# nebarnix/Project-Desert-Tortoise

Hardware: AMD Instinct MI355X
Metric: IQ Msamples/s end-to-end (WAV→minorframes), 1-GPU + %HBM roofline (higher is better)
Workload: dtype f32

## Files before the change

include/pdt_dev.h:

```cpp
#ifndef PDT_DEV_H
#define PDT_DEV_H
#include <stdint.h>
#ifdef __cplusplus
extern "C" {
#endif
int pdt_dev_set(const char *name, const char *value);
struct pdt_ctx;
unsigned long long pdt_dev_span_rows(const struct pdt_ctx *ctx, unsigned *n_exits_out, unsigned long long max);
int pdt_dev_ddc(int device, uint32_t in_rate, int decim, double offset_hz, int sample_format, const void *x_dev, long long lo, long long hi,
                uint64_t n_out, uint64_t g0, void *out_dev);
#ifdef __cplusplus
}
#endif
#endif
```

project-desert-tortoise_amd/__init__.py:

```python
from __future__ import annotations

import collections
import ctypes as C
import os
import struct

import numpy as np

_HERE = os.path.dirname(os.path.abspath(__file__))
LIBPDT_PATH = os.environ.get("PDT_LIBPDT_PATH") or os.path.join(_HERE, "csrc", "libpdt.so")
LIBSYNTH_PATH = os.path.join(_HERE, "synth", "libpdtsynth.so")

MODE_POES, MODE_ARGOS = 0, 1
SAMPLER_GARDNER, SAMPLER_MM = 0, 1
CHAIN_FILE, CHAIN_LIVE = 0, 1
ST_PLL, ST_LOCK, ST_FIR, ST_AGC, ST_SYM, ST_SYMIDX, ST_BITS, ST_BITSYM, ST_AGC_RAW, ST_ANALYTIC, ST_CHANNEL = range(11)
FMT_PCM16, FMT_F32, FMT_REAL_PCM16, FMT_REAL_F32 = range(4)


FMT_WB_PCM16, FMT_WB_F32, FMT_WB_CU8, FMT_WB_CS8 = range(16, 20)


class PdtError(RuntimeError):
    pass
# ... 238 lines not shown
    "pdt_demod_pcm16", "pdt_demod_device", "pdt_demod_f32", "pdt_demod_device_f32", "pdt_demod_batch_device", "pdt_num_frames", "pdt_frames", "pdt_get_stats",
    "pdt_format_frames", "pdt_read_stage", "pdt_stage_len", "pdt_kernel_times", "pdt_make_lpf",
    "pdt_wav_parse_header", "pdt_time_axis", "pdt_stage_bytesync", "pdt_tip_check", "pdt_tip_frames",
    "pdt_stream_begin", "pdt_stream_push_pcm16", "pdt_stream_push_f32", "pdt_stream_end", "pdt_stream_frames",
    "pdt_keep_quality", "pdt_chunk_reports", "pdt_stage_manchester", "pdt_stage_fir", "pdt_stage_agc", "pdt_stage_squelch", "pdt_stage_pll", "pdt_stage_gardner", "pdt_stage_static_gain", "pdt_stage_mm",
    "pdt_keep_presquelch", "pdt_keep_pll", "pdt_stage_bytesync_from", "pdt_demod_fd", "pdt_format_records", "pdt_stream_retained", "pdt_host_math", "pdt_get_device",
    "pdt_write_frames", "pdt_write_records", "pdt_demod_file", "pdt_set_loop_params", "pdt_set_progress",
    "pdt_set_real_input", "pdt_demod_real", "pdt_demod_device_real", "pdt_stream_push_real", "pdt_host_analytic",
    "pdt_set_channel", "pdt_demod_channel", "pdt_demod_device_channel", "pdt_demod_channels_device", "pdt_demod_channels", "pdt_stream_push_channel", "pdt_host_ddc",
    "pdt_survey", "pdt_survey_device", "pdt_survey_spectrum", "pdt_host_survey",
    "pdt_bursts", "pdt_bursts_device", "pdt_burst_carriers", "pdt_waterfall_rows", "pdt_bursts_shape", "pdt_burst_peaks", "pdt_host_bursts",
    "pdt_device_math", "pdt_device_math_layout",
    "pdt_burst_windows", "pdt_demod_windows_device", "pdt_demod_windows", "pdt_demod_windows_held",
    "pdt_tones", "pdt_tones_batch", "pdt_host_tones",
]
DEV_SYMBOLS = ["pdt_dev_set", "pdt_dev_span_rows", "pdt_dev_ddc"]

_lib = None


def _share_torch_hip_runtime():
    import importlib.util
    import sys
    if "torch" in sys.modules:
        return
    try:
        spec = importlib.util.find_spec("torch")
    except (ImportError, ValueError):
        return
    if spec is None or not spec.submodule_search_locations:
        return
# ... 77 lines not shown
    L.pdt_stage_fir.argtypes = [C.c_void_p, C.c_void_p, C.c_uint64, C.c_void_p, C.c_void_p]
    L.pdt_stage_fir.restype = C.c_int
    L.pdt_keep_quality.argtypes = [C.c_void_p, C.c_int]
    L.pdt_keep_quality.restype = C.c_int
    L.pdt_keep_pll.argtypes = [C.c_void_p, C.c_int]
    L.pdt_keep_pll.restype = C.c_int
    L.pdt_chunk_reports.argtypes = [C.c_void_p, C.c_void_p, C.c_uint64]
    L.pdt_chunk_reports.restype = C.c_uint64
    L.pdt_set_progress.argtypes = [C.c_void_p, C.c_void_p, C.c_void_p]
    L.pdt_tip_check.argtypes = [C.c_void_p, C.POINTER(TipSummary)]
    L.pdt_tip_frames.argtypes = [C.c_void_p, C.c_void_p, C.c_uint64]
    L.pdt_tip_frames.restype = C.c_uint64
    L.pdt_write_frames.argtypes = [C.c_void_p, C.c_int, C.POINTER(C.c_uint64)]
    L.pdt_write_records.argtypes = [C.c_void_p, C.c_uint64, C.c_int, C.POINTER(C.c_uint64)]
    L.pdt_dev_set.argtypes = [C.c_char_p, C.c_char_p]
    L.pdt_set_loop_params.argtypes = [C.c_void_p, C.POINTER(LoopParams)]
    L.pdt_demod_file.argtypes = [C.c_void_p, C.c_int, C.c_uint64, C.c_uint64, C.c_int, C.c_int, C.POINTER(C.c_uint64)]
    L.pdt_set_real_input.argtypes = [C.c_void_p, C.c_double]
    L.pdt_demod_real.argtypes = [C.c_void_p, C.c_void_p, C.c_uint64, C.c_int]
    L.pdt_demod_device_real.argtypes = [C.c_void_p, C.c_void_p, C.c_uint64, C.c_int]
    L.pdt_stream_push_real.argtypes = [C.c_void_p, C.c_void_p, C.c_uint64, C.c_int, C.POINTER(C.c_uint64)]
    L.pdt_host_analytic.argtypes = [C.c_uint32, C.c_double, C.c_void_p, C.c_uint64, C.c_int, C.c_void_p]
    L.pdt_set_channel.argtypes = [C.c_void_p, C.c_int, C.c_double]
    L.pdt_demod_channel.argtypes = [C.c_void_p, C.c_void_p, C.c_uint64, C.c_int]
    L.pdt_demod_device_channel.argtypes = [C.c_void_p, C.c_void_p, C.c_uint64, C.c_int]
    L.pdt_demod_channels_device.argtypes = [C.POINTER(C.c_void_p), C.c_int, C.c_void_p, C.c_uint64, C.c_int]
    L.pdt_demod_channels.argtypes = [C.POINTER(C.c_void_p), C.c_int, C.c_void_p, C.c_uint64, C.c_int]
    L.pdt_stream_push_channel.argtypes = [C.c_void_p, C.c_void_p, C.c_uint64, C.c_int, C.POINTER(C.c_uint64)]
    L.pdt_host_ddc.argtypes = [C.c_uint32, C.c_int, C.c_double, C.c_void_p, C.c_uint64, C.c_int, C.c_void_p]
    L.pdt_dev_ddc.argtypes = [C.c_int, C.c_uint32, C.c_int, C.c_double, C.c_int, C.c_void_p, C.c_longlong, C.c_longlong, C.c_uint64, C.c_uint64, C.c_void_p]
# ... 326 lines not shown
        c, cap = _tone_cfg(cfg)
        out, count = np.zeros(max(cap, 1), dtype=TONE_DTYPE), C.c_int(0)
        _check(self._L.pdt_tones(self._h, C.byref(c) if c else None, out.ctypes.data, cap, C.byref(count)), "pdt_tones")
        return out[:count.value]

    def device_math(self, fn: int, records: np.ndarray) -> np.ndarray:
        dt, nin, nout = device_math_layout(fn)
        a = np.ascontiguousarray(records)
        if a.dtype != dt or a.size % nin:
            raise PdtError(f"pdt_device_math({fn}): records of {nin} x {dt} wanted, got {a.dtype} x {a.shape}")
        n = a.size // nin
        out = np.empty((n, nout), dtype=dt)
        _check(self._L.pdt_device_math(self._h, fn, a.ctypes.data, n, out.ctypes.data), "pdt_device_math")
        return out

    def demod_device(self, dev_ptr: int, nframes: int):
        _check(self._L.pdt_demod_device(self._h, C.c_void_p(dev_ptr), nframes), "pdt_demod_device")
        return self

    def bytesync(self, bits: np.ndarray):
        b = np.ascontiguousarray(bits, dtype=np.uint8)
        _check(self._L.pdt_stage_bytesync(self._h, b.ctypes.data, b.size), "pdt_stage_bytesync")
        return self

    def _dt(self):
        return np.dtype("<f8") if (self.mode == MODE_ARGOS and not self.chain) else np.dtype("<f4")

    def stage_manchester(self, symbols: np.ndarray, resync_threshold: float, state: "ManchesterState | None" = None):
        a = np.ascontiguousarray(symbols, dtype=self._dt())
        bits = np.zeros(a.size + 4, dtype=np.uint8)
# ... 315 lines not shown
```

project-desert-tortoise_amd/csrc/pdt_api.hip:

```cpp
#include "pdt_rt.h"
#include "pdt_analytic.h"
#include "pdt_ddc.h"
#include "pdt_survey.h"
#include "pdt_bursts.h"
#include "pdt_tone.h"

#include <pthread.h>
#include <sched.h>
#include <sys/mman.h>
#include <sys/stat.h>
#include <sys/syscall.h>

namespace pdtrt {
PDT_CHAIN_INSTANCES(extern, float)
PDT_CHAIN_INSTANCES(extern, double)
std::atomic<long long> g_alloc_ns{0};
hipError_t analytic_launch(hipStream_t st, int fmt, const void *x, long long lo, long long hi, unsigned long long n_out, unsigned long long g0,
                           uint32_t step, const float *tab_dev, void *out);
size_t survey_part_floats(uint64_t nseg, int nfft);
hipError_t survey_launch(hipStream_t st, int fmt, const void *x, uint64_t nseg, int nfft, const float *win, const float *tw, float *part, float *out);
int survey_plan(const pdt_survey_cfg *cfg, double mode_range_hz, double channel_rate, uint64_t nframes, int cap, pdt::SurveyPlan *p);
int survey_carriers(const float *P, const pdt::SurveyPlan &p, double in_rate, pdt_carrier *found);
hipError_t waterfall_launch(hipStream_t st, int fmt, const void *x, uint64_t nrows, int rows_per, int nfft, const float *win, const float *tw, float *rows);
hipError_t row_peaks_launch(hipStream_t st, const float *rows, uint64_t nrows, int nfft, float level, int gb, void *peaks, int *counts);
// ... 30 lines not shown
    if (const char *e = get("PDT_PLL_BLOCK")) pll_block = atoi(e);
    if (const char *e = get("PDT_HBM_LIMIT_MB")) hbm_limit_mb = std::max(1ll, atoll(e));
    if (const char *e = get("PDT_BURST_SLAB_ROWS")) burst_slab_rows = std::max(1ll, atoll(e));
    if (const char *e = get("PDT_WINDOW_PIECE")) window_piece = std::max(1ll, atoll(e));
    if (const char *e = get("PDT_SCOUT_SYMS")) scout_syms = std::max(16, atoi(e));
    if (const char *e = get("PDT_FIR_WG_PER_CU")) fir_wg_per_cu = std::min(4096, std::max(1, atoi(e)));
    if (const char *e = get("PDT_INGEST_THREADS")) ingest_threads = std::min(128, std::max(1, atoi(e)));
    if (const char *e = get("PDT_INGEST_SPAN_MB")) ingest_span_mb = std::min(256, std::max(1, atoi(e)));
    if (const char *e = get("PDT_INGEST_STREAMS")) ingest_streams = std::min(4, std::max(1, atoi(e)));
    if (const char *e = get("PDT_INGEST_DIRECT")) ingest_direct = atoi(e) ? 1 : 0;
    if (const char *e = get("PDT_INGEST_NUMA")) ingest_numa = atoi(e) ? 1 : 0;
    if (const char *e = get("PDT_FIX_PASSES")) fix_passes = atoi(e);
    if (const char *e = get("PDT_GSEG")) gseg = std::min(64, std::max(2, atoi(e)));
    if (const char *e = get("PDT_GSPAN")) gspan = std::min(256, std::max(1, atoi(e)));
    if (const char *e = get("PDT_GSPAN_CAP")) gspan_cap = std::max(64, atoi(e));
    fir_generic = get("PDT_FIR_GENERIC") != nullptr;
    mix_unfused = get("PDT_MIX_UNFUSED") != nullptr;
    quality_inline = get("PDT_QUALITY_INLINE") != nullptr;
    gardner_nostride = get("PDT_GARDNER_NOSTRIDE") != nullptr;
    gemit_groups = get("PDT_GEMIT_GROUPS") != nullptr;
    agc_unfused = get("PDT_AGC_UNFUSED") != nullptr;
    manch_3pass = get("PDT_MANCH_3PASS") != nullptr;
    sync_serial = get("PDT_SYNC_SERIAL") != nullptr;
    agc_lanes = get("PDT_AGC_LANES") != nullptr;
    no_excl = get("PDT_NO_EXCL") != nullptr;
    gardner_onebuf = get("PDT_GARDNER_ONEBUF") != nullptr;
    gardner_noring = get("PDT_GARDNER_NORING") != nullptr;
    ema_noguess = get("PDT_EMA_NOGUESS") != nullptr;
    gardner_sequential = get("PDT_GARDNER_SEQUENTIAL") != nullptr;
    seg_sequential = get("PDT_SEG_SEQUENTIAL") != nullptr;
// ... 575 lines not shown
{
    if (!ctx || ctx->gspan_nrows <= 0 || !ctx->gspan_rows.p) return 0;
    const unsigned long long n = (unsigned long long)ctx->gspan_nrows, m = std::min(n, max);
    if (n_exits_out && m) {
        std::vector<GardnerSpanRow> rows((size_t)m);
        if (hipSetDevice(ctx->cfg.device) != hipSuccess ||
            hipMemcpy(rows.data(), ctx->gspan_rows.p, (size_t)m * sizeof(GardnerSpanRow), hipMemcpyDeviceToHost) != hipSuccess) {
            (void)hipGetLastError();
            return 0;
        }
        for (size_t k = 0; k < (size_t)m; k++) n_exits_out[k] = rows[k].n;
    }
    return n;
}

int pdt_dev_ddc(int device, uint32_t in_rate, int decim, double offset_hz, int sample_format, const void *x_dev, long long lo, long long hi,
                uint64_t n_out, uint64_t g0, void *out_dev)
{
    if (in_rate == 0 || decim < DDC_MIN_DECIM || decim > DDC_MAX_DECIM || !ddc_fmt(sample_format) || !x_dev || !out_dev) return PDT_ERR_ARG;
    if (!(std::isfinite(offset_hz) && std::fabs(offset_hz) < 0.5 * (double)in_rate)) return PDT_ERR_ARG;
    HIP_TRY(hipSetDevice(device));
    const std::vector<float> taps = ddc_taps(decim);
    std::vector<float> tab(2 * AN_TAB);
    analytic_table(tab.data());
    DevBuf dtaps, dtab;
    auto run = [&]() -> int {
        int rc;
        if ((rc = dtaps.ensure(taps.size() * sizeof(float) + 16)) || (rc = dtab.ensure(tab.size() * sizeof(float) + 16))) return rc;
        HIP_TRY(hipMemcpy(dtaps.p, taps.data(), taps.size() * sizeof(float), hipMemcpyHostToDevice));
        HIP_TRY(hipMemcpy(dtab.p, tab.data(), tab.size() * sizeof(float), hipMemcpyHostToDevice));
// ... 192 lines not shown
    if (argos_twin) ctx->axis_f.init(1 / (float)cfg->sample_rate);
    ctx->axis_d.init(1.0 / (double)cfg->sample_rate);
    ctx->counted = true;
    g_open_contexts.fetch_add(1);
    *out = ctx;
    return PDT_OK;
}

void pdt_close(pdt_ctx *ctx)
{
    if (!ctx) return;
    (void)hipSetDevice(ctx->cfg.device);
    DevBuf *bufs[] = { &ctx->pcm, &ctx->pll, &ctx->lock, &ctx->fir, &ctx->agc, &ctx->sym, &ctx->symidx, &ctx->bits, &ctx->bitsym,
                       &ctx->hits, &ctx->frames, &ctx->taps, &ctx->mag, &ctx->seams_pll, &ctx->seams_agc, &ctx->scal, &ctx->lockinfo,
                       &ctx->term, &ctx->seams_ema, &ctx->gtable, &ctx->gentries, &ctx->gcand,
                       &ctx->gmfirst, &ctx->stiles, &ctx->gsegmap, &ctx->gsegstart, &ctx->gbands, &ctx->gclist, &ctx->gspan_keys, &ctx->gspan_tails, &ctx->gspan_rows, &ctx->gspan_items, &ctx->gspan_ctl, &ctx->gspan_recs, &ctx->gcentries, &ctx->gflags, &ctx->agc_maps, &ctx->pll_head, &ctx->taps_rot, &ctx->pll_scratch, &ctx->tip, &ctx->stream_in, &ctx->sync_scr, &ctx->agc_raw, &ctx->agc_ckpt, &ctx->pll_ckpt, &ctx->packs_dev, &ctx->seg_dev, &ctx->lt_theta, &ctx->lt_phi,
                       &ctx->avgph, &ctx->term_ap, &ctx->seams_q, &ctx->chunkinfo, &ctx->an_tab, &ctx->analytic, &ctx->halo.buf[0], &ctx->halo.buf[1],
                       &ctx->ddc_taps, &ctx->channel, &ctx->survey_win, &ctx->survey_tw, &ctx->survey_part, &ctx->survey_out,
                       &ctx->bursts_rows, &ctx->bursts_peaks, &ctx->bursts_counts, &ctx->win_table, &ctx->tone_table, &ctx->tone_out };
    for (DevBuf *b : bufs) b->release();
    for (hipEvent_t e : ctx->event_pool) (void)hipEventDestroy(e);
    if (ctx->pinned) (void)hipHostFree(ctx->pinned);
    if (ctx->qual_pin) (void)hipHostFree(ctx->qual_pin);
    if (ctx->packs_pin) (void)hipHostFree(ctx->packs_pin);
    if (ctx->ingest_pin) (void)hipHostFree(ctx->ingest_pin);
    for (hipEvent_t e : ctx->ingest_ev) (void)hipEventDestroy(e);
    if (ctx->ev_ingest) (void)hipEventDestroy(ctx->ev_ingest);
    if (ctx->copy_stream) (void)hipStreamDestroy(ctx->copy_stream);
    for (hipEvent_t e : ctx->span_ev) (void)hipEventDestroy(e);
    for (int q = 0; q < 3; q++) {
        if (ctx->ev_ingest_more[q]) (void)hipEventDestroy(ctx->ev_ingest_more[q]);
// ... 1743 lines not shown
```

project-desert-tortoise_amd/csrc/pdt_chain.inc:

```
#include "pdt_rt.h"

namespace pdtrt {
PDT_WIDE_INSTANCES(extern, float)
PDT_WIDE_INSTANCES(extern, double)

template <typename T> int finish_capture(pdt_ctx *ctx, uint64_t n, const FinishArgs &FA)
{
    const bool argos = FA.argos, need_lock = FA.need_lock, fuse_mix = FA.fuse_mix;
    const long long N = FA.N, n_out = FA.n_out, chunk = FA.chunk, chunk_out = FA.chunk_out, first = FA.first, first_out = FA.first_out,
                    sym_cap = FA.sym_cap;
    const int interp = FA.interp, ntaps = FA.ntaps;
    const uint32_t hit_cap = FA.hit_cap, frame_cap = FA.frame_cap;
    const SyncParams &SP = FA.SP;
    const T Fs = (T)ctx->cfg.sample_rate;
    StreamCarry *seg = ctx->sc.active ? &ctx->sc : nullptr;
    FrameRec *d_frames = (FrameRec *)ctx->frames.p;
    (void)first_out;
    if (!ctx->pending || ctx->pend_n != n) return PDT_ERR_STATE;
    ctx->pending = false;
    pdt_ctx *lead = ctx->leader ? ctx->leader : ctx;
    if (seg && seg->in_place && !ctx->tune.sync_block) {
        for (;;) {
            const hipError_t e = hipEventQuery(lead->ev1);
            if (e == hipSuccess) break;
// ... 1155 lines not shown
                    PDT_LAUNCH(PDT_GTM_THREADS, (k_gardner_table_merge<PDT_GTAB_WIN>), dim3((unsigned)n_tab, parts), dim3(PDT_GTM_THREADS), 0, st,
                                       (const float *)d_agc, GP, GD, n_tab, (const unsigned *)ctx->gcand.p,
                                       (const GardnerBand *)ctx->gbands.p, (const unsigned *)ctx->gclist.p,
                                       (unsigned *)ctx->gtable.p, d_sc->gstats);
                }
                if (GD.span > 1) {
                    const unsigned cap_keys = ctx->tune.gspan_cap ? (unsigned)ctx->tune.gspan_cap
                                                                  : (unsigned)std::min<long long>(std::max<long long>(n_tab * 128, 1ll << 20), 1ll << 28);
                    const size_t cap_items = (size_t)cap_keys / PDT_GSUB_KEYS + (size_t)n_tab + 1;
                    if ((rc = ctx->gspan_keys.ensure((size_t)cap_keys * sizeof(unsigned)))) return rc;
                    if ((rc = ctx->gspan_tails.ensure((size_t)cap_keys * sizeof(unsigned)))) return rc;
                    if ((rc = ctx->gspan_recs.ensure((size_t)cap_keys * (size_t)(GD.span - 1) * sizeof(GardnerSpanRec)))) return rc;
                    if ((rc = ctx->gspan_rows.ensure((size_t)n_tab * sizeof(GardnerSpanRow)))) return rc;
                    if ((rc = ctx->gspan_items.ensure(cap_items * sizeof(GardnerSpanItem)))) return rc;
                    if ((rc = ctx->gspan_ctl.ensure(sizeof(GardnerSpanCtl)))) return rc;
                    PL.memset_async(ctx->gspan_ctl.p, 0, sizeof(GardnerSpanCtl));
                    PDT_LAUNCH(256, k_gardner_span_keys, dim3((unsigned)n_tab), dim3(256), 0, st, GD, n_tab, (const unsigned *)ctx->gcand.p,
                                       (GardnerBand *)ctx->gbands.p, (const unsigned *)ctx->gclist.p, (const unsigned *)ctx->gtable.p,
                                       (unsigned *)ctx->gspan_keys.p, cap_keys, (GardnerSpanRow *)ctx->gspan_rows.p,
                                       (GardnerSpanItem *)ctx->gspan_items.p, (GardnerSpanCtl *)ctx->gspan_ctl.p);
                    const unsigned walkers = (unsigned)std::min<long long>(n_tab / PDT_GSUB + 64, 256ll * 16);
                    PDT_LAUNCH(64, (k_gardner_span_walk<PDT_GSUB_WIN>), dim3(walkers), dim3(64), 0, st, (const float *)d_agc, GP, GD,
                                       (const unsigned *)ctx->gspan_keys.p, (const GardnerSpanItem *)ctx->gspan_items.p,
                                       (GardnerSpanCtl *)ctx->gspan_ctl.p, (unsigned *)ctx->gspan_tails.p, (GardnerSpanRec *)ctx->gspan_recs.p);
                    PDT_LAUNCH(128, k_gardner_span_join, dim3((unsigned)n_tab), dim3(128), 0, st, GD, n_tab, (const unsigned *)ctx->gcand.p,
                                       (const GardnerBand *)ctx->gbands.p, (const unsigned *)ctx->gclist.p, (unsigned *)ctx->gtable.p,
                                       (const unsigned *)ctx->gspan_keys.p, (const unsigned *)ctx->gspan_tails.p,
                                       (const GardnerSpanRow *)ctx->gspan_rows.p, d_sc->gstats);
                }
            }
            L.end();
            int G = (n_groups < 8000) ? 32 : 64;
            if (ctx->tune.gseg) G = ctx->tune.gseg;
            const long long n_seg = (n_groups + G - 1) / G;
            if ((rc = ctx->gsegmap.ensure((size_t)n_seg * (size_t)(2 * GD.n_q) * sizeof(GardnerSegCell)))) return rc;
            if ((rc = ctx->gsegstart.ensure((size_t)n_seg * sizeof(GardnerSegStart)))) return rc;
            L.begin("gardner_chain");
            PL.memset_async(ctx->gsegstart.p, 0, (size_t)n_seg * sizeof(GardnerSegStart));
            PDT_LAUNCH(1024, k_gardner_segmap, dim3((unsigned)n_seg), dim3(1024), 0, st, (const unsigned *)ctx->gtable.p, GD, n_groups,
                               G, (GardnerSegCell *)ctx->gsegmap.p, (const GardnerBand *)ctx->gbands.p);
            const int n_ranges = (!seg && n_groups >= 8192 && GD.span == 1 && !ctx->tune.chain_one_range) ? 4 : 1;
            if ((rc = ctx->gchain.ensure(sizeof(GardnerChainState)))) return rc;
            const bool side = n_ranges > 1;
// ... 698 lines not shown
```

project-desert-tortoise_amd/csrc/pdt_kernels_back.h:

```cpp
#pragma once
#include "pdt_device_math.h"

namespace pdt {

template <typename T> struct alignas(16) Vec16 {
    static constexpr int N = 16 / sizeof(T);
    T v[N];
};

template <typename T> struct GardnerParams {
    T step, kp, lim;
    long long n_total;
    long long chunk_out;
    int argos_heap;
    unsigned long long argos_field_bits;
    int argos_even;
};

template <typename T>
__device__ __forceinline__ T gardner_beyond(const T *__restrict__ in, const T *__restrict__ lock, const GardnerParams<T> &P,
                                            long long c, long long n_cur, long long idx)
{
    const long long C = P.chunk_out;
    if (idx < C)
// ... 1208 lines not shown
            const unsigned cnt = (unsigned)((int)x_cnt[o] + extra[q]);
            const unsigned cell = gardner_encode_exit(D, x_q[o], x_il[o], cnt);
            if (cell == PDT_GTAB_MISS) atomicAdd(&stats[0], 1u);
            row[my_k[l]] = cell;
        }
    }
}

#define PDT_GSPAN_BITMAP_WORDS 8192
#define PDT_GSUB 1
#define PDT_GSUB_WIN 2048
#define PDT_GSUB_KEYS (64 / PDT_GSUB)
struct GardnerSpanRow { unsigned off, n; };
struct GardnerSpanItem { unsigned row, first, cnt; };
struct GardnerSpanRec { float ns, prev, half; unsigned count; };
struct GardnerSpanCtl { unsigned long long keys; unsigned items, cursor, overflow, pad_; };

__device__ __forceinline__ void k_gardner_span_keys(GardnerDomain D, long long n_rows, const unsigned *__restrict__ cand_k,
                                                    GardnerBand *__restrict__ bands, const unsigned *__restrict__ clist,
                                                    const unsigned *__restrict__ table, unsigned *__restrict__ keys,
                                                    unsigned cap_keys, GardnerSpanRow *__restrict__ rows,
                                                    GardnerSpanItem *__restrict__ items, GardnerSpanCtl *__restrict__ ctl)
{
    __shared__ unsigned s_bits[PDT_GSPAN_BITMAP_WORDS];
    __shared__ unsigned s_scan[256];
    __shared__ unsigned s_off, s_item;
    const long long r = blockIdx.x;
    if (r >= n_rows) return;
    const long long c0 = r * D.span;
    const GardnerBand bd = bands[r];
    const unsigned *cand = bd.listed ? (clist + (size_t)r * PDT_GTAB_LIST) : cand_k;
    const unsigned *row = table + (size_t)r * (size_t)(2 * D.n_q);
    const int tid = threadIdx.x;
    const int n_words = (2 * D.n_q + 31) >> 5;
    const unsigned kmask = (1u << D.idx_bits) - 1u;
    for (int t = tid; t < n_words; t += 256) s_bits[t] = 0u;
    __syncthreads();
    for (int j = bd.j_lo + tid; j < bd.j_hi; j += 256) {
        const unsigned cell = row[(c0 == 0) ? 0u : cand[j]];
        if (cell != PDT_GTAB_MISS) {
            const unsigned k1 = cell & kmask;
            atomicOr(&s_bits[k1 >> 5], 1u << (k1 & 31u));
        }
// ... 21 lines not shown
        if (off == ~0u) atomicAdd(&ctl->overflow, 1u);
        else s_item = atomicAdd(&ctl->items, (total + (unsigned)PDT_GSUB_KEYS - 1u) / (unsigned)PDT_GSUB_KEYS);
        s_off = off;
    }
    __syncthreads();
    const unsigned off = s_off;
    if (off == ~0u) {
        if (tid == 0) {
            GardnerSpanRow rw;
            rw.off = 0; rw.n = ~0u;
            rows[r] = rw;
            GardnerBand nb = bd;
            nb.k_lo = 1u; nb.k_hi = 0u;
            bands[r] = nb;
        }
        return;
    }
    unsigned at = off + s_scan[tid] - mine;
    for (int t = w0; t < w1; t++) {
        unsigned bits = s_bits[t];
        while (bits) {
            const int b = __ffs((int)bits) - 1;
            bits &= bits - 1u;
            keys[at++] = ((unsigned)t << 5) + (unsigned)b;
        }
    }
    for (unsigned q = tid; q < (total + (unsigned)PDT_GSUB_KEYS - 1u) / (unsigned)PDT_GSUB_KEYS; q += 256u) {
        GardnerSpanItem it;
        it.row = (unsigned)r;
        it.first = off + (unsigned)PDT_GSUB_KEYS * q;
        it.cnt = (total - (unsigned)PDT_GSUB_KEYS * q < (unsigned)PDT_GSUB_KEYS) ? total - (unsigned)PDT_GSUB_KEYS * q : (unsigned)PDT_GSUB_KEYS;
        items[s_item + q] = it;
    }
    if (tid == 0) {
        GardnerSpanRow rw;
        rw.off = off; rw.n = total;
        rows[r] = rw;
    }
}

#define PDT_GSUB_OUT 64
template <int WIN, int NSUB, bool EMIT>
__device__ __forceinline__ void gardner_sub_chunk(float *win, const float *__restrict__ in, const GardnerParams<float> &P,
                                                  const long long (&c_sub)[NSUB], GardnerLane &L, float *__restrict__ sym,
                                                  long long *__restrict__ symidx, long long sym_at, long long sym_cap,
                                                  float *o_val = nullptr, unsigned *o_idx = nullptr )
{
    constexpr int SUBW = 64 / NSUB;
    const int lane = (int)threadIdx.x;
    const int mysub = lane / SUBW;
    float *ov = o_val + mysub * PDT_GSUB_OUT;
    unsigned *oi = o_idx + mysub * PDT_GSUB_OUT;
// ... 127 lines not shown


template <int WIN>
__device__ __forceinline__ void k_gardner_span_walk(const float *__restrict__ in, GardnerParams<float> P, GardnerDomain D,
                                                    const unsigned *__restrict__ keys, const GardnerSpanItem *__restrict__ items,
                                                    GardnerSpanCtl *__restrict__ ctl, unsigned *__restrict__ tails,
                                                    GardnerSpanRec *__restrict__ recs )
{
    __shared__ __attribute__((aligned(16))) float win[PDT_GSUB * WIN];
    __shared__ float s_ref[3];
    __shared__ unsigned s_next;
    const int lane = threadIdx.x;
    const int mysub = lane / PDT_GSUB_KEYS, sublane = lane % PDT_GSUB_KEYS;
    const float nT = (float)P.chunk_out;
    const unsigned n_items = ctl->items;
    for (;;) {
        __syncthreads();
        if (lane == 0) s_next = atomicAdd(&ctl->cursor, (unsigned)PDT_GSUB);
        __syncthreads();
        const unsigned q0 = s_next;
        if (q0 >= n_items) break;
        long long c_sub[PDT_GSUB];
        GardnerSpanItem mine = items[q0];
#pragma unroll
        for (int u = 0; u < PDT_GSUB; u++) {
            const GardnerSpanItem it = (q0 + (unsigned)u < n_items) ? items[q0 + u] : items[q0];
            c_sub[u] = (long long)it.row * D.span + 1;
            if (mysub == u) {
                mine = it;
                if (q0 + (unsigned)u >= n_items) mine.cnt = 0;
// ... 11 lines not shown
        __syncthreads();
        if (!L.active) { L.ns = s_ref[0]; L.prev = s_ref[1]; L.half = s_ref[2]; }
        for (int g = 1; g < D.span; g++) {
            long long cc[PDT_GSUB];
#pragma unroll
            for (int u = 0; u < PDT_GSUB; u++) cc[u] = c_sub[u] + (g - 1);
            if (L.active) {
                GardnerSpanRec rc;
                rc.ns = L.ns; rc.prev = L.prev; rc.half = L.half; rc.count = L.count;
                recs[(size_t)(mine.first + sublane) * (size_t)(D.span - 1) + (size_t)(g - 1)] = rc;
            }
            gardner_sub_chunk<WIN, PDT_GSUB, false>(win, in, P, cc, L, nullptr, nullptr, 0, 0);
            if (g + 1 < D.span) L.ns = L.ns - nT;
        }
        if (L.active) tails[mine.first + sublane] = gardner_encode_exit(D, L.q_last, L.i_last, L.count);
    }
}

#define PDT_GEMIT_SUB_WIN 512
template <int WIN>
__device__ __forceinline__ void k_gardner_emit_first(const float *__restrict__ in, GardnerParams<float> P, GardnerDomain D,
                                                     long long n_rows, const GardnerEntry<float> *__restrict__ entries,
                                                     const unsigned *__restrict__ keys, const GardnerSpanRow *__restrict__ rows,
                                                     const GardnerSpanRec *__restrict__ recs,
                                                     GardnerEntry<float> *__restrict__ centries, unsigned char *__restrict__ flags,
                                                     float *__restrict__ sym, long long *__restrict__ symidx, long long sym_cap,
                                                     long long g_first = 0 )
{
    __shared__ __attribute__((aligned(16))) float win[4 * WIN];
    const int lane = threadIdx.x;
// ... 71 lines not shown
    for (int u = 0; u < 4; u++)
        if (mysub == u) { my_c = c_sub[u]; mine_live = live[u]; }
    const GardnerEntry<float> e = centries[my_c];
    GardnerLane L;
    L.ns = e.ns; L.prev = e.prev; L.half = e.half; L.q_last = 0; L.i_last = 0; L.count = 0; L.k = 0;
    L.active = mine_live;
    __shared__ float o_val[4 * PDT_GSUB_OUT];
    __shared__ unsigned o_idx[4 * PDT_GSUB_OUT];
    gardner_sub_chunk<WIN, 4, true>(win, in, P, c_sub, L, sym, symidx, e.offset, sym_cap, o_val, o_idx);
}

__device__ __forceinline__ void k_gardner_span_join(GardnerDomain D, long long n_rows, const unsigned *__restrict__ cand_k,
                                                    const GardnerBand *__restrict__ bands, const unsigned *__restrict__ clist,
                                                    unsigned *__restrict__ table, const unsigned *__restrict__ keys,
                                                    const unsigned *__restrict__ tails, const GardnerSpanRow *__restrict__ rows,
                                                    unsigned *__restrict__ stats )
{
    const long long r = blockIdx.x;
    if (r >= n_rows) return;
    const GardnerSpanRow rw = rows[r];
    if (rw.n == ~0u) return;
    const long long c0 = r * D.span;
    const GardnerBand bd = bands[r];
    const unsigned *cand = bd.listed ? (clist + (size_t)r * PDT_GTAB_LIST) : cand_k;
    unsigned *row = table + (size_t)r * (size_t)(2 * D.n_q);
    const unsigned kmask = (1u << D.idx_bits) - 1u;
    for (int j = bd.j_lo + (int)threadIdx.x; j < bd.j_hi; j += (int)blockDim.x) {
        const unsigned k = (c0 == 0) ? 0u : cand[j];
        const unsigned cell = row[k];
        if (cell == PDT_GTAB_MISS) continue;
        const unsigned k1 = cell & kmask;
        unsigned lo = 0, hi = rw.n;
        while (lo < hi) {
            const unsigned mid = (lo + hi) >> 1;
            if (keys[rw.off + mid] < k1) lo = mid + 1;
            else hi = mid;
        }
        unsigned out = PDT_GTAB_MISS;
        if (lo < rw.n && keys[rw.off + lo] == k1) {
            const unsigned tail = tails[rw.off + lo];
            if (tail != PDT_GTAB_MISS) {
                const unsigned cnt = (cell >> D.idx_bits) + (tail >> D.idx_bits);
                if (cnt < (1u << (32 - D.idx_bits)) - 1u) out = (tail & kmask) | (cnt << D.idx_bits);
            }
        }
        if (out == PDT_GTAB_MISS) atomicAdd(&stats[0], 1u);
        row[k] = out;
    }
}

__device__ __forceinline__ unsigned gardner_cell(const unsigned *__restrict__ table, size_t stride, const GardnerBand &b,
                                                 long long c, unsigned key)
{
    const unsigned cell = table[(size_t)c * stride + key];
    return (key >= b.k_lo && key <= b.k_hi) ? cell : PDT_GTAB_MISS;
}

struct GardnerSegCell { unsigned next, count; };
struct GardnerSegStart { unsigned key; unsigned hopped; long long offset; };

__device__ __forceinline__ void k_gardner_segmap(const unsigned *__restrict__ table, GardnerDomain D, long long n_groups,
                                                          int G, GardnerSegCell *__restrict__ segmap,
// ... 1315 lines not shown
```

project-desert-tortoise_amd/csrc/pdt_rt.h:

```cpp
#ifndef PDT_RT_H
#define PDT_RT_H
#include <hip/hip_runtime.h>
#include <math.h>
#include <stdio.h>
#include <stdlib.h>
#include <string.h>

#include <errno.h>
#include <fcntl.h>
#include <unistd.h>

#include <algorithm>
#include <functional>
#include <map>
#include <mutex>
#include <atomic>
#include <chrono>
#include <memory>
#include <new>
#include <string>
#include <thread>
#include <type_traits>
#include <vector>

// ... 211 lines not shown
        }
        return true;
    }
};
#define PDT_LAUNCH(TB, KERNEL, grid, block, shmem, stream, ...) \
    PL.launch<&KERNEL, TB>(#KERNEL, grid, block, shmem, PL.side_of(stream), __VA_ARGS__)

}
using namespace pdtrt;

struct Tuning {
    double band_pad = 0.0, pll_warm_scale = 1.0, head_taus = 0.0, agc_k = 0.0, pll_warm_s = 0.0, agc_warm_s = 0.0;
    double overlap_split[8] = { 0, 0, 0, 0, 0, 0, 0, 0 };
    long long hbm_limit_mb = 0, window_piece = 0, burst_slab_rows = 0;
    int ingest_direct = -1, ingest_numa = -1;
    int scout_syms = 0, gspan = 0, gspan_cap = 0, ingest_threads = 0, ingest_span_mb = 0, ingest_streams = 0, overlap_segments = 0, overlap_min_mb = 0, fir_wg_per_cu = 0, agc_tpb = 0, gseg = 0, pll_block = 0, fix_passes = 2;
    bool fir_generic = false, mix_unfused = false, quality_inline = false, gemit_groups = false, agc_unfused = false, no_excl = false, gardner_onebuf = false, gardner_noring = false, gardner_sequential = false, seg_sequential = false, agc_lanes = false, overlap = true, debug_overlap = false, chain_one_range = false, ema_noguess = false, debug_sync = false, pll_noshort = false, pll_nockpt = false, pll_noconsensus = false, pll_notail = false, seg_plain = false, sync_block = false, gardner_nostride = false, manch_3pass = false, sync_serial = false;
    void load();
};

struct StreamCarry {
    bool active = false;
    bool final_seg = false;
    bool in_place = false;
    uint64_t place_align = 0;
    bool quality = false;
    long long first = 0;
    uint64_t origin = 0;
    bool have_norm = false;
    double norm_factor = 0, gain = 0;
    bool locked = false;
    double phase = 0, freq = 0, avg = 0, locksig = 0, sweep = 0;
// ... 44 lines not shown
    uint64_t left = 0, pending = 0, in = 0, out = 0;
};

struct pdt_ctx {
    pdt_config cfg;
    pdt_loop_params lp = {};
    Tuning tune;
    StreamCarry sc;
    int elem;
    uint32_t interp, ntaps;
    hipStream_t stream = nullptr;
    bool own_stream = false;
    hipEvent_t ev0 = nullptr, ev1 = nullptr, ev_fork = nullptr, ev_join = nullptr;
    hipStream_t stream2 = nullptr;

    DevBuf pcm, pll, lock, fir, agc, sym, symidx, bits, bitsym, hits, frames, taps, mag, seams_pll, seams_agc, scal, lockinfo, term, seams_ema, gtable, gentries, gcand, gmfirst, stiles, gsegmap, gsegstart, gbands, gclist, gneed, gchain, gspan_keys, gspan_tails, gspan_rows, gspan_items, gspan_ctl, gspan_recs, gcentries, gflags, agc_maps, pll_head, taps_rot, pll_scratch, tip, sync_scr, agc_raw, agc_ckpt, pll_ckpt;
    bool counted = false;
    bool keep_agc_raw = false;
    bool keep_quality = false;
    bool keep_pll_asked = false;
    bool keep_pll = true;
    DevBuf avgph, term_ap, seams_q, chunkinfo;
    struct PllInject {
        bool active = false, started = false, locked = false;
        double phase = 0, freq = 0, avg = 0, locksig = 0, sweep = 0;
    } inj;
    long long last_pll_block = 0;
    void *qual_pin = nullptr;
    size_t qual_pin_cap = 0;
    uint64_t pend_chunks = 0;
    std::vector<pdt::ChunkInfo> chunk_host;
    uint64_t report_samples = 0;
    pdt_progress_fn progress_fn = nullptr;
    void *progress_user = nullptr;
    long long gcand_key = -1;
    int gardner_mode = 0;
    long long gspan_nrows = 0;
    const void *pcm_dev = nullptr;
    int pcm_fmt = 0;

    std::vector<unsigned char> taps_host;
    uint64_t n_samples = 0, n_out = 0;
    std::vector<pdt_frame> frames_host;
    std::vector<pdt_tip_frame> tip_host;
    uint32_t frames_on_device = 0;
    bool have_frames = false;
    Plan plan;
    DevBuf packs_dev;
    void *packs_pin = nullptr;
    size_t packs_pin_cap = 0;
    pdt_ctx *leader = nullptr;
    int batch_hint = 1;
// ... 278 lines not shown
```

Before: 51490.

## Add fused per-row Gardner span kernel handling keys, walk and join for small rows

Adds a new persistent k_gardner_span_row kernel that pulls rows from an atomic cursor. For each row it builds the key set in shared memory, walks the span and joins the results back into the table, all within one workgroup. Rows whose key count exceeds a limit (default 64) are appended to a list. The existing keys and join kernels then loop over only that list using capped grids, and walk returns early when there are no items. This is meant to replace three full per-row launches and the global item indirection for the common small-key case, at the cost of an extra pass and an extra launch for rows that overflow. It is enabled by default and can be disabled with PDT_GSPAN_SPLIT; a diagnostic span_paths API is also added.

Result: faster. 52130, median of 6 (+1.2%).

```diff
diff --git a/include/pdt_dev.h b/include/pdt_dev.h
--- a/include/pdt_dev.h
+++ b/include/pdt_dev.h
@@ -7,6 +7,7 @@
 int pdt_dev_set(const char *name, const char *value);
 struct pdt_ctx;
 unsigned long long pdt_dev_span_rows(const struct pdt_ctx *ctx, unsigned *n_exits_out, unsigned long long max);
+int pdt_dev_span_paths(const struct pdt_ctx *ctx, unsigned long long *n_row_kernel, unsigned long long *n_listed);
 int pdt_dev_ddc(int device, uint32_t in_rate, int decim, double offset_hz, int sample_format, const void *x_dev, long long lo, long long hi,
                 uint64_t n_out, uint64_t g0, void *out_dev);
 #ifdef __cplusplus
diff --git a/project-desert-tortoise_amd/__init__.py b/project-desert-tortoise_amd/__init__.py
--- a/project-desert-tortoise_amd/__init__.py
+++ b/project-desert-tortoise_amd/__init__.py
@@ -276,7 +276,7 @@
     "pdt_burst_windows", "pdt_demod_windows_device", "pdt_demod_windows", "pdt_demod_windows_held",
     "pdt_tones", "pdt_tones_batch", "pdt_host_tones",
 ]
-DEV_SYMBOLS = ["pdt_dev_set", "pdt_dev_span_rows", "pdt_dev_ddc"]
+DEV_SYMBOLS = ["pdt_dev_set", "pdt_dev_span_rows", "pdt_dev_span_paths", "pdt_dev_ddc"]
 
 _lib = None
 
@@ -384,6 +384,9 @@
     L.pdt_write_frames.argtypes = [C.c_void_p, C.c_int, C.POINTER(C.c_uint64)]
     L.pdt_write_records.argtypes = [C.c_void_p, C.c_uint64, C.c_int, C.POINTER(C.c_uint64)]
     L.pdt_dev_set.argtypes = [C.c_char_p, C.c_char_p]
+    L.pdt_dev_span_rows.argtypes = [C.c_void_p, C.c_void_p, C.c_uint64]
+    L.pdt_dev_span_rows.restype = C.c_uint64
+    L.pdt_dev_span_paths.argtypes = [C.c_void_p, C.POINTER(C.c_uint64), C.POINTER(C.c_uint64)]
     L.pdt_set_loop_params.argtypes = [C.c_void_p, C.POINTER(LoopParams)]
     L.pdt_demod_file.argtypes = [C.c_void_p, C.c_int, C.c_uint64, C.c_uint64, C.c_int, C.c_int, C.POINTER(C.c_uint64)]
     L.pdt_set_real_input.argtypes = [C.c_void_p, C.c_double]
@@ -740,6 +743,18 @@
         _check(self._L.pdt_device_math(self._h, fn, a.ctypes.data, n, out.ctypes.data), "pdt_device_math")
         return out
 
+    def span_rows(self) -> np.ndarray:
+        n = int(self._L.pdt_dev_span_rows(self._h, None, 0))
+        out = np.zeros(n, dtype=np.uint32)
+        if n:
+            self._L.pdt_dev_span_rows(self._h, out.ctypes.data, n)
+        return out
+
+    def span_paths(self) -> tuple[int, int]:
+        a, b = C.c_uint64(0), C.c_uint64(0)
+        _check(self._L.pdt_dev_span_paths(self._h, C.byref(a), C.byref(b)), "pdt_dev_span_paths")
+        return int(a.value), int(b.value)
+
     def demod_device(self, dev_ptr: int, nframes: int):
         _check(self._L.pdt_demod_device(self._h, C.c_void_p(dev_ptr), nframes), "pdt_demod_device")
         return self
diff --git a/project-desert-tortoise_amd/csrc/pdt_api.hip b/project-desert-tortoise_amd/csrc/pdt_api.hip
--- a/project-desert-tortoise_amd/csrc/pdt_api.hip
+++ b/project-desert-tortoise_amd/csrc/pdt_api.hip
@@ -68,6 +68,8 @@
     if (const char *e = get("PDT_GSEG")) gseg = std::min(64, std::max(2, atoi(e)));
     if (const char *e = get("PDT_GSPAN")) gspan = std::min(256, std::max(1, atoi(e)));
     if (const char *e = get("PDT_GSPAN_CAP")) gspan_cap = std::max(64, atoi(e));
+    if (const char *e = get("PDT_GSPAN_ROWKEYS")) gspan_rowkeys = std::min(64, std::max(1, atoi(e)));
+    gspan_split = get("PDT_GSPAN_SPLIT") != nullptr;
     fir_generic = get("PDT_FIR_GENERIC") != nullptr;
     mix_unfused = get("PDT_MIX_UNFUSED") != nullptr;
     quality_inline = get("PDT_QUALITY_INLINE") != nullptr;
@@ -673,6 +675,21 @@
     return n;
 }
 
+int pdt_dev_span_paths(const pdt_ctx *ctx, unsigned long long *n_row_kernel, unsigned long long *n_listed)
+{
+    if (!ctx || !n_row_kernel || !n_listed) return PDT_ERR_ARG;
+    *n_row_kernel = *n_listed = 0;
+    if (ctx->gspan_nrows <= 0 || !ctx->gspan_ctl.p) return PDT_OK;
+    const unsigned long long n = (unsigned long long)ctx->gspan_nrows;
+    if (!ctx->gspan_by_row) { *n_listed = n; return PDT_OK; }
+    GardnerSpanCtl ctl;
+    HIP_TRY(hipSetDevice(ctx->cfg.device));
+    HIP_TRY(hipMemcpy(&ctl, ctx->gspan_ctl.p, sizeof ctl, hipMemcpyDeviceToHost));
+    *n_listed = std::min<unsigned long long>(ctl.listed, n);
+    *n_row_kernel = n - *n_listed;
+    return PDT_OK;
+}
+
 int pdt_dev_ddc(int device, uint32_t in_rate, int decim, double offset_hz, int sample_format, const void *x_dev, long long lo, long long hi,
                 uint64_t n_out, uint64_t g0, void *out_dev)
 {
@@ -895,7 +912,7 @@
     DevBuf *bufs[] = { &ctx->pcm, &ctx->pll, &ctx->lock, &ctx->fir, &ctx->agc, &ctx->sym, &ctx->symidx, &ctx->bits, &ctx->bitsym,
                        &ctx->hits, &ctx->frames, &ctx->taps, &ctx->mag, &ctx->seams_pll, &ctx->seams_agc, &ctx->scal, &ctx->lockinfo,
                        &ctx->term, &ctx->seams_ema, &ctx->gtable, &ctx->gentries, &ctx->gcand,
-                       &ctx->gmfirst, &ctx->stiles, &ctx->gsegmap, &ctx->gsegstart, &ctx->gbands, &ctx->gclist, &ctx->gspan_keys, &ctx->gspan_tails, &ctx->gspan_rows, &ctx->gspan_items, &ctx->gspan_ctl, &ctx->gspan_recs, &ctx->gcentries, &ctx->gflags, &ctx->agc_maps, &ctx->pll_head, &ctx->taps_rot, &ctx->pll_scratch, &ctx->tip, &ctx->stream_in, &ctx->sync_scr, &ctx->agc_raw, &ctx->agc_ckpt, &ctx->pll_ckpt, &ctx->packs_dev, &ctx->seg_dev, &ctx->lt_theta, &ctx->lt_phi,
+                       &ctx->gmfirst, &ctx->stiles, &ctx->gsegmap, &ctx->gsegstart, &ctx->gbands, &ctx->gclist, &ctx->gspan_keys, &ctx->gspan_tails, &ctx->gspan_rows, &ctx->gspan_items, &ctx->gspan_ctl, &ctx->gspan_recs, &ctx->gspan_list, &ctx->gcentries, &ctx->gflags, &ctx->agc_maps, &ctx->pll_head, &ctx->taps_rot, &ctx->pll_scratch, &ctx->tip, &ctx->stream_in, &ctx->sync_scr, &ctx->agc_raw, &ctx->agc_ckpt, &ctx->pll_ckpt, &ctx->packs_dev, &ctx->seg_dev, &ctx->lt_theta, &ctx->lt_phi,
                        &ctx->avgph, &ctx->term_ap, &ctx->seams_q, &ctx->chunkinfo, &ctx->an_tab, &ctx->analytic, &ctx->halo.buf[0], &ctx->halo.buf[1],
                        &ctx->ddc_taps, &ctx->channel, &ctx->survey_win, &ctx->survey_tw, &ctx->survey_part, &ctx->survey_out,
                        &ctx->bursts_rows, &ctx->bursts_peaks, &ctx->bursts_counts, &ctx->win_table, &ctx->tone_table, &ctx->tone_out };
diff --git a/project-desert-tortoise_amd/csrc/pdt_chain.inc b/project-desert-tortoise_amd/csrc/pdt_chain.inc
--- a/project-desert-tortoise_amd/csrc/pdt_chain.inc
+++ b/project-desert-tortoise_amd/csrc/pdt_chain.inc
@@ -1193,19 +1193,31 @@
                     if ((rc = ctx->gspan_rows.ensure((size_t)n_tab * sizeof(GardnerSpanRow)))) return rc;
                     if ((rc = ctx->gspan_items.ensure(cap_items * sizeof(GardnerSpanItem)))) return rc;
                     if ((rc = ctx->gspan_ctl.ensure(sizeof(GardnerSpanCtl)))) return rc;
+                    if ((rc = ctx->gspan_list.ensure((size_t)n_tab * sizeof(unsigned)))) return rc;
                     PL.memset_async(ctx->gspan_ctl.p, 0, sizeof(GardnerSpanCtl));
-                    PDT_LAUNCH(256, k_gardner_span_keys, dim3((unsigned)n_tab), dim3(256), 0, st, GD, n_tab, (const unsigned *)ctx->gcand.p,
+                    const unsigned walkers = (unsigned)std::min<long long>(n_tab / PDT_GSUB + 64, 256ll * 16);
+                    const bool by_row = !ctx->tune.gspan_split;
+                    ctx->gspan_by_row = by_row;
+                    const unsigned *d_list = by_row ? (const unsigned *)ctx->gspan_list.p : nullptr;
+                    if (by_row)
+                        PDT_LAUNCH(64, (k_gardner_span_row<PDT_GSUB_WIN>), dim3(walkers), dim3(64), 0, st, (const float *)d_agc, GP, GD, n_tab,
+                                           (const unsigned *)ctx->gcand.p, (GardnerBand *)ctx->gbands.p, (const unsigned *)ctx->gclist.p,
+                                           (unsigned *)ctx->gtable.p, (unsigned *)ctx->gspan_keys.p, cap_keys, (GardnerSpanRow *)ctx->gspan_rows.p,
+                                           (GardnerSpanCtl *)ctx->gspan_ctl.p, (unsigned *)ctx->gspan_tails.p, (GardnerSpanRec *)ctx->gspan_recs.p,
+                                           (unsigned *)ctx->gspan_list.p, (unsigned)ctx->tune.gspan_rowkeys, d_sc->gstats);
+                    const unsigned key_grid = by_row ? (unsigned)std::min<long long>(n_tab, 1024) : (unsigned)n_tab;
+                    const unsigned join_grid = by_row ? (unsigned)std::min<long long>(n_tab, 2048) : (unsigned)n_tab;
+                    PDT_LAUNCH(256, k_gardner_span_keys, dim3(key_grid), dim3(256), 0, st, GD, n_tab, (const unsigned *)ctx->gcand.p,
                                        (GardnerBand *)ctx->gbands.p, (const unsigned *)ctx->gclist.p, (const unsigned *)ctx->gtable.p,
                                        (unsigned *)ctx->gspan_keys.p, cap_keys, (GardnerSpanRow *)ctx->gspan_rows.p,
-                                       (GardnerSpanItem *)ctx->gspan_items.p, (GardnerSpanCtl *)ctx->gspan_ctl.p);
-                    const unsigned walkers = (unsigned)std::min<long long>(n_tab / PDT_GSUB + 64, 256ll * 16);
+                                       (GardnerSpanItem *)ctx->gspan_items.p, (GardnerSpanCtl *)ctx->gspan_ctl.p, d_list);
                     PDT_LAUNCH(64, (k_gardner_span_walk<PDT_GSUB_WIN>), dim3(walkers), dim3(64), 0, st, (const float *)d_agc, GP, GD,
                                        (const unsigned *)ctx->gspan_keys.p, (const GardnerSpanItem *)ctx->gspan_items.p,
                                        (GardnerSpanCtl *)ctx->gspan_ctl.p, (unsigned *)ctx->gspan_tails.p, (GardnerSpanRec *)ctx->gspan_recs.p);
-                    PDT_LAUNCH(128, k_gardner_span_join, dim3((unsigned)n_tab), dim3(128), 0, st, GD, n_tab, (const unsigned *)ctx->gcand.p,
+                    PDT_LAUNCH(128, k_gardner_span_join, dim3(join_grid), dim3(128), 0, st, GD, n_tab, (const unsigned *)ctx->gcand.p,
                                        (const GardnerBand *)ctx->gbands.p, (const unsigned *)ctx->gclist.p, (unsigned *)ctx->gtable.p,
                                        (const unsigned *)ctx->gspan_keys.p, (const unsigned *)ctx->gspan_tails.p,
-                                       (const GardnerSpanRow *)ctx->gspan_rows.p, d_sc->gstats);
+                                       (const GardnerSpanRow *)ctx->gspan_rows.p, d_sc->gstats, (const GardnerSpanCtl *)ctx->gspan_ctl.p, d_list);
                 }
             }
             L.end();
diff --git a/project-desert-tortoise_amd/csrc/pdt_kernels_back.h b/project-desert-tortoise_amd/csrc/pdt_kernels_back.h
--- a/project-desert-tortoise_amd/csrc/pdt_kernels_back.h
+++ b/project-desert-tortoise_amd/csrc/pdt_kernels_back.h
@@ -1246,19 +1246,26 @@
 struct GardnerSpanRow { unsigned off, n; };
 struct GardnerSpanItem { unsigned row, first, cnt; };
 struct GardnerSpanRec { float ns, prev, half; unsigned count; };
-struct GardnerSpanCtl { unsigned long long keys; unsigned items, cursor, overflow, pad_; };
+struct GardnerSpanCtl {
+    unsigned long long keys;
+    unsigned items, cursor, overflow;
+    unsigned row_cursor, listed, pad_;
+};
 
 __device__ __forceinline__ void k_gardner_span_keys(GardnerDomain D, long long n_rows, const unsigned *__restrict__ cand_k,
                                                     GardnerBand *__restrict__ bands, const unsigned *__restrict__ clist,
                                                     const unsigned *__restrict__ table, unsigned *__restrict__ keys,
                                                     unsigned cap_keys, GardnerSpanRow *__restrict__ rows,
-                                                    GardnerSpanItem *__restrict__ items, GardnerSpanCtl *__restrict__ ctl)
+                                                    GardnerSpanItem *__restrict__ items, GardnerSpanCtl *__restrict__ ctl,
+                                                    const unsigned *__restrict__ list )
 {
     __shared__ unsigned s_bits[PDT_GSPAN_BITMAP_WORDS];
     __shared__ unsigned s_scan[256];
     __shared__ unsigned s_off, s_item;
-    const long long r = blockIdx.x;
-    if (r >= n_rows) return;
+    const long long n_work = list ? (long long)ctl->listed : n_rows;
+    for (long long w = blockIdx.x; w < n_work; w += gridDim.x) {
+    const long long r = list ? (long long)list[w] : w;
+    __syncthreads();
     const long long c0 = r * D.span;
     const GardnerBand bd = bands[r];
     const unsigned *cand = bd.listed ? (clist + (size_t)r * PDT_GTAB_LIST) : cand_k;
@@ -1310,7 +1317,7 @@
             nb.k_lo = 1u; nb.k_hi = 0u;
             bands[r] = nb;
         }
-        return;
+        continue;
     }
     unsigned at = off + s_scan[tid] - mine;
     for (int t = w0; t < w1; t++) {
@@ -1332,6 +1339,7 @@
         GardnerSpanRow rw;
         rw.off = off; rw.n = total;
         rows[r] = rw;
+    }
     }
 }
 
@@ -1489,6 +1497,7 @@
     const int mysub = lane / PDT_GSUB_KEYS, sublane = lane % PDT_GSUB_KEYS;
     const float nT = (float)P.chunk_out;
     const unsigned n_items = ctl->items;
+    if (n_items == 0) return;
     for (;;) {
         __syncthreads();
         if (lane == 0) s_next = atomicAdd(&ctl->cursor, (unsigned)PDT_GSUB);
@@ -1530,6 +1539,178 @@
             if (g + 1 < D.span) L.ns = L.ns - nT;
         }
         if (L.active) tails[mine.first + sublane] = gardner_encode_exit(D, L.q_last, L.i_last, L.count);
+    }
+}
+
+#define PDT_GROW_KEYS 64
+#define PDT_GROW_BATCH 8
+#define PDT_GROW_CELLS 32
+typedef unsigned __attribute__((may_alias)) pdt_u32_alias;
+template <int WIN>
+__device__ __forceinline__ void k_gardner_span_row(const float *__restrict__ in, GardnerParams<float> P, GardnerDomain D, long long n_rows,
+                                                   const unsigned *__restrict__ cand_k, GardnerBand *__restrict__ bands,
+                                                   const unsigned *__restrict__ clist, unsigned *__restrict__ table,
+                                                   unsigned *__restrict__ keys, unsigned cap_keys, GardnerSpanRow *__restrict__ rows,
+                                                   GardnerSpanCtl *__restrict__ ctl, unsigned *__restrict__ tails,
+                                                   GardnerSpanRec *__restrict__ recs, unsigned *__restrict__ list,
+                                                   unsigned max_keys , unsigned *__restrict__ stats )
+{
+    static_assert(WIN >= 4 * PDT_GROW_KEYS, "the window buffer also holds the key list");
+    __shared__ __attribute__((aligned(16))) float win[WIN];
+    __shared__ unsigned s_next;
+    pdt_u32_alias *wbits = reinterpret_cast<pdt_u32_alias *>(win);
+    pdt_u32_alias *wkeys = wbits + (WIN - PDT_GROW_KEYS);
+    const int lane = threadIdx.x;
+    const int n_words = (2 * D.n_q + 31) >> 5;
+    const bool fits = n_words <= WIN - PDT_GROW_KEYS;
+    const unsigned kmask = (1u << D.idx_bits) - 1u;
+    const float nT = (float)P.chunk_out;
+    if (max_keys > (unsigned)PDT_GROW_KEYS) max_keys = (unsigned)PDT_GROW_KEYS;
+    for (;;) {
+        __syncthreads();
+        if (lane == 0) s_next = atomicAdd(&ctl->row_cursor, 1u);
+        __syncthreads();
+        const unsigned r = (unsigned)__builtin_amdgcn_readfirstlane((int)s_next);
+        if ((long long)r >= n_rows) break;
+        const long long c0 = (long long)r * D.span;
+        const GardnerBand bd = bands[r];
+        const unsigned *cand = bd.listed ? (clist + (size_t)r * PDT_GTAB_LIST) : cand_k;
+        unsigned *row = table + (size_t)r * (size_t)(2 * D.n_q);
+        unsigned total = ~0u;
+        if (fits) {
+            for (int t = lane; t < n_words; t += 64) wbits[t] = 0u;
+            __syncthreads();
+            const int per = (n_words + 63) / 64;
+            const int w0 = lane * per, w1 = (w0 + per < n_words) ? w0 + per : n_words;
+            unsigned mine = 0, incl = 0;
+            total = 0u;
+            for (int j0 = bd.j_lo; j0 < bd.j_hi && total <= max_keys; j0 += 64 * PDT_GROW_CELLS) {
+                const int j1 = (j0 + 64 * PDT_GROW_CELLS < bd.j_hi) ? j0 + 64 * PDT_GROW_CELLS : bd.j_hi;
+                for (int j = j0 + lane; j < j1; j += 64 * PDT_GROW_BATCH) {
+                    unsigned kk[PDT_GROW_BATCH], cl[PDT_GROW_BATCH];
+#pragma unroll
+                    for (int u = 0; u < PDT_GROW_BATCH; u++)
+                        kk[u] = (j + 64 * u < j1) ? ((c0 == 0) ? 0u : cand[j + 64 * u]) : ~0u;
+#pragma unroll
+                    for (int u = 0; u < PDT_GROW_BATCH; u++) cl[u] = (kk[u] != ~0u) ? row[kk[u]] : PDT_GTAB_MISS;
+#pragma unroll
+                    for (int u = 0; u < PDT_GROW_BATCH; u++)
+                        if (cl[u] != PDT_GTAB_MISS) {
+                            const unsigned k1 = cl[u] & kmask;
+                            if ((int)(k1 >> 5) < n_words) atomicOr(&wbits[k1 >> 5], 1u << (k1 & 31u));
+                        }
+                }
+                __syncthreads();
+                mine = 0;
+                for (int t = w0; t < w1; t++) mine += (unsigned)__popc(wbits[t]);
+                incl = mine;
+#pragma unroll
+                for (int d = 1; d < 64; d <<= 1) {
+                    const unsigned v = (unsigned)__shfl_up((int)incl, d, 64);
+                    if (lane >= d) incl += v;
+                }
+                total = (unsigned)__builtin_amdgcn_readlane((int)incl, 63);
+            }
+            if (total <= max_keys) {
+                unsigned at = incl - mine;
+                for (int t = w0; t < w1; t++) {
+                    unsigned bits = wbits[t];
+                    while (bits) {
+                        const int b = __ffs((int)bits) - 1;
+                        bits &= bits - 1u;
+                        wkeys[at++] = ((unsigned)t << 5) + (unsigned)b;
+                    }
+                }
+            } else
+                total = ~0u;
+        }
+        if (total == ~0u) {
+            if (lane == 0) list[atomicAdd(&ctl->listed, 1u)] = r;
+            continue;
+        }
+        const unsigned n_keys = (unsigned)__builtin_amdgcn_readfirstlane((int)total);
+        __syncthreads();
+        const unsigned my_key = ((unsigned)lane < n_keys) ? wkeys[lane] : 0u;
+        unsigned off = 0u;
+        if (lane == 0) {
+            const unsigned long long got = atomicAdd(&ctl->keys, (unsigned long long)n_keys);
+            off = (got + n_keys <= (unsigned long long)cap_keys) ? (unsigned)got : ~0u;
+            if (off == ~0u) atomicAdd(&ctl->overflow, 1u);
+        }
+        off = (unsigned)__builtin_amdgcn_readfirstlane((int)off);
+        if (off == ~0u) {
+            if (lane == 0) {
+                GardnerSpanRow rw;
+                rw.off = 0; rw.n = ~0u;
+                rows[r] = rw;
+                GardnerBand nb = bd;
+                nb.k_lo = 1u; nb.k_hi = 0u;
+                bands[r] = nb;
+            }
+            continue;
+        }
+        if ((unsigned)lane < n_keys) keys[off + lane] = my_key;
+        if (lane == 0) {
+            GardnerSpanRow rw;
+            rw.off = off; rw.n = n_keys;
+            rows[r] = rw;
+        }
+        if (n_keys == 0u) continue;
+        GardnerLane L;
+        L.q_last = 0; L.i_last = 0; L.count = 0; L.k = 0;
+        L.active = (unsigned)lane < n_keys;
+        L.ns = L.prev = L.half = 0;
+        const long long c1 = c0 + 1;
+        if (L.active) gardner_entry_from_candidate(in, P, D, c1, (int)my_key, L.ns, L.prev, L.half);
+        {
+            const float ns0 = __shfl(L.ns, 0, 64), prev0 = __shfl(L.prev, 0, 64), half0 = __shfl(L.half, 0, 64);
+            if (!L.active) { L.ns = ns0; L.prev = prev0; L.half = half0; }
+        }
+        for (int g = 1; g < D.span; g++) {
+            const long long cc[1] = { c1 + (g - 1) };
+            if (L.active) {
+                GardnerSpanRec rc;
+                rc.ns = L.ns; rc.prev = L.prev; rc.half = L.half; rc.count = L.count;
+                recs[(size_t)(off + lane) * (size_t)(D.span - 1) + (size_t)(g - 1)] = rc;
+            }
+            gardner_sub_chunk<WIN, 1, false>(win, in, P, cc, L, nullptr, nullptr, 0, 0);
+            if (g + 1 < D.span) L.ns = L.ns - nT;
+        }
+        const unsigned tail = L.active ? gardner_encode_exit(D, L.q_last, L.i_last, L.count) : PDT_GTAB_MISS;
+        if (L.active) tails[off + lane] = tail;
+        __syncthreads();
+        wbits[lane] = L.active ? my_key : ~0u;
+        wbits[PDT_GROW_KEYS + lane] = tail;
+        __syncthreads();
+        for (int j = bd.j_lo + lane; j < bd.j_hi; j += 64 * PDT_GROW_BATCH) {
+            unsigned kk[PDT_GROW_BATCH], cl[PDT_GROW_BATCH], pos[PDT_GROW_BATCH];
+#pragma unroll
+            for (int u = 0; u < PDT_GROW_BATCH; u++) kk[u] = (j + 64 * u < bd.j_hi) ? ((c0 == 0) ? 0u : cand[j + 64 * u]) : ~0u;
+#pragma unroll
+            for (int u = 0; u < PDT_GROW_BATCH; u++) {
+                cl[u] = (kk[u] != ~0u) ? row[kk[u]] : PDT_GTAB_MISS;
+                pos[u] = 0u;
+            }
+#pragma unroll
+            for (unsigned step = PDT_GROW_KEYS / 2; step; step >>= 1)
+#pragma unroll
+                for (int u = 0; u < PDT_GROW_BATCH; u++)
+                    if (wbits[pos[u] + step - 1u] < (cl[u] & kmask)) pos[u] += step;
+#pragma unroll
+            for (int u = 0; u < PDT_GROW_BATCH; u++) {
+                if (cl[u] == PDT_GTAB_MISS) continue;
+                unsigned out = PDT_GTAB_MISS;
+                if (wbits[pos[u]] == (cl[u] & kmask)) {
+                    const unsigned tl = wbits[PDT_GROW_KEYS + pos[u]];
+                    if (tl != PDT_GTAB_MISS) {
+                        const unsigned cnt = (cl[u] >> D.idx_bits) + (tl >> D.idx_bits);
+                        if (cnt < (1u << (32 - D.idx_bits)) - 1u) out = (tl & kmask) | (cnt << D.idx_bits);
+                    }
+                }
+                if (out == PDT_GTAB_MISS) atomicAdd(&stats[0], 1u);
+                row[kk[u]] = out;
+            }
+        }
     }
 }
 
@@ -1631,12 +1812,14 @@
                                                     const GardnerBand *__restrict__ bands, const unsigned *__restrict__ clist,
                                                     unsigned *__restrict__ table, const unsigned *__restrict__ keys,
                                                     const unsigned *__restrict__ tails, const GardnerSpanRow *__restrict__ rows,
-                                                    unsigned *__restrict__ stats )
-{
-    const long long r = blockIdx.x;
-    if (r >= n_rows) return;
+                                                    unsigned *__restrict__ stats ,
+                                                    const GardnerSpanCtl *__restrict__ ctl, const unsigned *__restrict__ list )
+{
+    const long long n_work = list ? (long long)ctl->listed : n_rows;
+    for (long long w = blockIdx.x; w < n_work; w += gridDim.x) {
+    const long long r = list ? (long long)list[w] : w;
     const GardnerSpanRow rw = rows[r];
-    if (rw.n == ~0u) return;
+    if (rw.n == ~0u) continue;
     const long long c0 = r * D.span;
     const GardnerBand bd = bands[r];
     const unsigned *cand = bd.listed ? (clist + (size_t)r * PDT_GTAB_LIST) : cand_k;
@@ -1663,6 +1846,7 @@
         }
         if (out == PDT_GTAB_MISS) atomicAdd(&stats[0], 1u);
         row[k] = out;
+    }
     }
 }
 
diff --git a/project-desert-tortoise_amd/csrc/pdt_rt.h b/project-desert-tortoise_amd/csrc/pdt_rt.h
--- a/project-desert-tortoise_amd/csrc/pdt_rt.h
+++ b/project-desert-tortoise_amd/csrc/pdt_rt.h
@@ -249,8 +249,8 @@
     double overlap_split[8] = { 0, 0, 0, 0, 0, 0, 0, 0 };
     long long hbm_limit_mb = 0, window_piece = 0, burst_slab_rows = 0;
     int ingest_direct = -1, ingest_numa = -1;
-    int scout_syms = 0, gspan = 0, gspan_cap = 0, ingest_threads = 0, ingest_span_mb = 0, ingest_streams = 0, overlap_segments = 0, overlap_min_mb = 0, fir_wg_per_cu = 0, agc_tpb = 0, gseg = 0, pll_block = 0, fix_passes = 2;
-    bool fir_generic = false, mix_unfused = false, quality_inline = false, gemit_groups = false, agc_unfused = false, no_excl = false, gardner_onebuf = false, gardner_noring = false, gardner_sequential = false, seg_sequential = false, agc_lanes = false, overlap = true, debug_overlap = false, chain_one_range = false, ema_noguess = false, debug_sync = false, pll_noshort = false, pll_nockpt = false, pll_noconsensus = false, pll_notail = false, seg_plain = false, sync_block = false, gardner_nostride = false, manch_3pass = false, sync_serial = false;
+    int scout_syms = 0, gspan = 0, gspan_cap = 0, gspan_rowkeys = 64, ingest_threads = 0, ingest_span_mb = 0, ingest_streams = 0, overlap_segments = 0, overlap_min_mb = 0, fir_wg_per_cu = 0, agc_tpb = 0, gseg = 0, pll_block = 0, fix_passes = 2;
+    bool gspan_split = false, fir_generic = false, mix_unfused = false, quality_inline = false, gemit_groups = false, agc_unfused = false, no_excl = false, gardner_onebuf = false, gardner_noring = false, gardner_sequential = false, seg_sequential = false, agc_lanes = false, overlap = true, debug_overlap = false, chain_one_range = false, ema_noguess = false, debug_sync = false, pll_noshort = false, pll_nockpt = false, pll_noconsensus = false, pll_notail = false, seg_plain = false, sync_block = false, gardner_nostride = false, manch_3pass = false, sync_serial = false;
     void load();
 };
 
@@ -325,7 +325,7 @@
     hipEvent_t ev0 = nullptr, ev1 = nullptr, ev_fork = nullptr, ev_join = nullptr;
     hipStream_t stream2 = nullptr;
 
-    DevBuf pcm, pll, lock, fir, agc, sym, symidx, bits, bitsym, hits, frames, taps, mag, seams_pll, seams_agc, scal, lockinfo, term, seams_ema, gtable, gentries, gcand, gmfirst, stiles, gsegmap, gsegstart, gbands, gclist, gneed, gchain, gspan_keys, gspan_tails, gspan_rows, gspan_items, gspan_ctl, gspan_recs, gcentries, gflags, agc_maps, pll_head, taps_rot, pll_scratch, tip, sync_scr, agc_raw, agc_ckpt, pll_ckpt;
+    DevBuf pcm, pll, lock, fir, agc, sym, symidx, bits, bitsym, hits, frames, taps, mag, seams_pll, seams_agc, scal, lockinfo, term, seams_ema, gtable, gentries, gcand, gmfirst, stiles, gsegmap, gsegstart, gbands, gclist, gneed, gchain, gspan_keys, gspan_tails, gspan_rows, gspan_items, gspan_ctl, gspan_recs, gspan_list, gcentries, gflags, agc_maps, pll_head, taps_rot, pll_scratch, tip, sync_scr, agc_raw, agc_ckpt, pll_ckpt;
     bool counted = false;
     bool keep_agc_raw = false;
     bool keep_quality = false;
@@ -347,6 +347,7 @@
     long long gcand_key = -1;
     int gardner_mode = 0;
     long long gspan_nrows = 0;
+    bool gspan_by_row = false;
     const void *pcm_dev = nullptr;
     int pcm_fmt = 0;
 
```
